# instance-based-loc/instance-based-loc

Hardware: AMD Instinct MI355X
Metric: query-frames localized/sec (embed+match+register) (higher is better)
Workload: dtype f16 (ViT MFMA operands, f32 accumulate) / f32+f64 (match, registration); 1 GPU; T: dinov2_vitb14 crops 224^2 (Q=7), 10000-instance memory (E=4), FPFH+RANSAC+coloured ICP on 5000-pt clouds, whole-memory evaluate; synthetic objects of extent U[0.15, 0.6] m on a 2.50 m grid (SURVEY 8d's U[0.2, 1.5] m re-scoped: its 5 000 points are too sparse to survive the radius-outlier removal); memory_instances=10000, points_per_object=5000, resident_feature_bytes_per_point=264, parallelism=frames-dp1+memory-replicated

## Files before the change

instance-based-loc_amd/csrc/reg_api.hip:

```cpp
#pragma clang fp contract(off)
#include <hip/hip_runtime.h>

#include <hipcub/hipcub.hpp>

#include <cctype>
#include <climits>
#include <cmath>
#include <cstdlib>
#include <cstring>
#include <string>
#include <vector>

#include "ibloc.h"
#include "reg_common.h"

#ifndef KNN_CELLS_NORMAL
#define KNN_CELLS_NORMAL 3.0
#endif
#ifndef KNN_CELLS_FEATURE
#define KNN_CELLS_FEATURE 5.0
#endif

#ifndef KNN_TILE_NORMAL
#define KNN_TILE_NORMAL 4
// ... 36 lines not shown
    bool auto0 = false;
};
static const DiagSwitch DIAG_SWITCHES[] = {
    {"knn_safety", nullptr},
    {"knn_rho", &RegDiag::knn_rho, 1, 4},
    {"knn_noguess", &RegDiag::knn_noguess},
    {"knn_debug", &RegDiag::knn_debug},
    {"feat_unfused", &RegDiag::feat_unfused},
    {"feat_valu", &RegDiag::feat_valu},
    {"feat_cand_cap", &RegDiag::feat_cand_cap, 1, INT_MAX, true},
    {"feat_p1_stride", &RegDiag::feat_p1_stride, 1},
    {"spfh_f64", &RegDiag::spfh_f64},
    {"spfh_qcap", &RegDiag::spfh_qcap, 1, INT_MAX, true},
    {"spfh_stats", &RegDiag::spfh_stats},
    {"eval_fullscan", &RegDiag::eval_fullscan},
    {"timing", &RegDiag::timing},
};

static const DiagSwitch* find_diag(const char* name) {
    for (const DiagSwitch& d : DIAG_SWITCHES)
        if (name && strcmp(name, d.name) == 0) return &d;
    return nullptr;
}

extern "C" int ibl_reg_ctx_set_diag(ibl_reg_ctx* ctx, const char* name, double value) {
    const DiagSwitch* d = find_diag(name);
    if (!ctx || !d || !std::isfinite(value)) return ibl_set_error(IBL_ERR_ARG, "ibl_reg_ctx_set_diag: null context, unknown switch or non-finite value");
    if (!d->field) ctx->diag.knn_safety = value;
    else if (d->auto0 && value == 0) ctx->diag.*d->field = 0;
    else ctx->diag.*d->field = (int)std::min(std::max(value, (double)d->lo), (double)d->hi);
// ... 381 lines not shown
```

instance-based-loc_amd/csrc/reg_common.h:

```cpp
#pragma once
#include <hip/hip_runtime.h>

#include <cstdint>

#include "ibl_common.h"

struct SegGrid {
    float minx, miny, minz, inv;
    int nx, ny, nz;
    int cell_base;
};

struct BatchGrid {
    const SegGrid* seg;
    const int* cell_start;
    const float4* sorted_pts;
    const int* order;
    int n_seg;
    const int* tile_base;
    const int* tile_seg;
    int n_tiles;
    int ts;
};

#define FM_P1_STRIDE 2

struct RegDiag {
    double knn_safety = 1.1;
    int knn_rho = 3;
    int knn_noguess = 0, knn_debug = 0;
    int feat_unfused = 0, feat_valu = 0, feat_cand_cap = 0;
    int feat_p1_stride = FM_P1_STRIDE;
    int spfh_f64 = 0, spfh_qcap = 0, spfh_stats = 0;
    int eval_fullscan = 0;
    int timing = 0;
};

struct ibl_reg_ctx {
    RegDiag diag;
    unsigned char* base = nullptr;
    int64_t size = 0;
    int64_t used = 0;
    int64_t high_water = 0;
    int device = 0;
    int* d_status = nullptr;
    unsigned char* pin = nullptr;
    int64_t pin_size = 0;
    int64_t pin_used = 0;
};
// ... 33 lines not shown
    } while (0)

#define IBL_ERR_ARENA (-5)
#define IBL_ERR_OVERFLOW (-6)

#define IBL_ST_GRID_OVERFLOW 1
#define IBL_ST_KNN_SLOWPATH 2
#define IBL_ST_FEAT_OVERFLOW 4
#define IBL_ST_RANSAC_OVERFLOW 8
#define IBL_ST_FEAT_REDONE 16
#define IBL_ST_RANSAC_REDONE 32

int ibl_build_batch_grid(ibl_reg_ctx* ctx, const float4* pts, const int* seg_off_dev, const int* seg_off_host, int n_seg,
                         float cell, int64_t max_cells, BatchGrid* out, hipStream_t s);
int ibl_build_batch_grid_bounded(ibl_reg_ctx* ctx, const float4* pts, const int* seg_off_dev, const int* seg_off_host, int n_seg,
                                 float cell, int64_t cells_bound, BatchGrid* out, hipStream_t s);
int ibl_build_tile_grid(ibl_reg_ctx* ctx, const float4* pts, const int* seg_off_dev, const int* seg_off_host, int n_seg,
                        const float* bbox_host, double radius, int max_nn, int ts, int64_t max_cells, BatchGrid* out, hipStream_t s);

int ibl_launch_bbox(const float4* pts, const int* seg_off_dev, int n_seg, float* bbox_dev, hipStream_t s);

struct FeatSources { const float4* normals[3]; const float* fpfh[3]; const float4* grad[3]; const unsigned short* split[3]; const float* norm[3]; };
struct FeatPair { int qkind, qsrc, qcnt, dkind, dsrc, dcnt, out, pad; };

int ibl_feat_search_mfma(ibl_reg_ctx* ctx, const FeatPair* d_pairs, int n_pairs, int max_q, const FeatSources& src, int* pair_idx,
                         float* pair_d2, const int* need_pos, const int* need_list, int out0, int64_t out_count, bool* overflow,
                         hipStream_t s);

int ibl_features_on_batch(ibl_reg_ctx* ctx, const float4* P, const int* seg_off_dev, const int* seg_off_host, int n_seg, const float* bbox_host, double voxel_size,
                          double grad_radius, int gq0, int gq1, float4* normals, float* fpfh, unsigned short* fpfh_split, float* fpfh_norm,
                          float4* grad, hipStream_t s);
// ... 173 lines not shown
```

instance-based-loc_amd/csrc/reg_grid.hip:

```cpp
#include <hip/hip_runtime.h>
#include <hipcub/hipcub.hpp>

#include <cstdlib>
#include <cstring>
#include <vector>

#include "reg_common.h"

__global__ __launch_bounds__(256) void ibl_bbox_kernel(const float4* __restrict__ pts, const int* __restrict__ seg_off,
                                                       float* __restrict__ bbox ) {
    const int s = blockIdx.x;
    const int b = seg_off[s], e = seg_off[s + 1];
    float mn[3] = {INFINITY, INFINITY, INFINITY}, mx[3] = {-INFINITY, -INFINITY, -INFINITY};
    for (int i = b + threadIdx.x; i < e; i += 256) {
        const float4 p = pts[i];
        mn[0] = fminf(mn[0], p.x); mn[1] = fminf(mn[1], p.y); mn[2] = fminf(mn[2], p.z);
        mx[0] = fmaxf(mx[0], p.x); mx[1] = fmaxf(mx[1], p.y); mx[2] = fmaxf(mx[2], p.z);
    }
    __shared__ float smn[3][256], smx[3][256];
    for (int a = 0; a < 3; ++a) { smn[a][threadIdx.x] = mn[a]; smx[a][threadIdx.x] = mx[a]; }
    __syncthreads();
    for (int st = 128; st >= 1; st >>= 1) {
        if (threadIdx.x < st)
            for (int a = 0; a < 3; ++a) {
// ... 21 lines not shown
    const float ex = b[3] - b[0], ey = b[4] - b[1], ez = b[5] - b[2];
    float c = cell;
    const float emax = fmaxf(ex, fmaxf(ey, ez));
    if (emax / 128.0f > c) c = emax / 128.0f;
    SegGrid g;
    g.minx = b[0]; g.miny = b[1]; g.minz = b[2];
    g.inv = 1.0f / c;
    g.nx = (int)floorf(ex * g.inv) + 1;
    g.ny = (int)floorf(ey * g.inv) + 1;
    g.nz = (int)floorf(ez * g.inv) + 1;
    g.cell_base = 0;
    return g;
}

__global__ __launch_bounds__(256) void ibl_grid_dims_kernel(const float* __restrict__ bbox, int n_seg, float cell, long long max_cells,
                                                            SegGrid* __restrict__ seg, int* __restrict__ total_cells, int* __restrict__ status) {
    __shared__ long long wave_sum[4];
    __shared__ long long carry;
    __shared__ int overflow_at;
    const int tid = threadIdx.x, lane = tid & 63, wave = tid >> 6;
    if (tid == 0) { carry = 0; overflow_at = -1; }
    __syncthreads();
    for (int base = 0; base < n_seg; base += 256) {
        const int s = base + tid;
        SegGrid g;
        long long cells = 0;
        if (s < n_seg) {
            g = seg_dims(bbox + s * 6, cell);
            cells = (long long)g.nx * g.ny * g.nz;
        }
        long long incl = cells;
#pragma unroll
        for (int off = 1; off < 64; off <<= 1) {
            const long long o = __shfl_up(incl, off, 64);
            if (lane >= off) incl += o;
        }
        if (lane == 63) wave_sum[wave] = incl;
        __syncthreads();
        long long before = carry;
        for (int w = 0; w < wave; ++w) before += wave_sum[w];
        const long long excl = before + incl - cells;
        if (s < n_seg) {
            if (excl + cells > max_cells) atomicMin(&overflow_at, s);
            g.cell_base = (int)excl;
            seg[s] = g;
        }
        __syncthreads();
        if (tid == 0) carry += wave_sum[0] + wave_sum[1] + wave_sum[2] + wave_sum[3];
        __syncthreads();
        if (overflow_at >= 0) break;
    }
    if (overflow_at >= 0) {
        if (tid == 0) {
            long long base = seg[overflow_at].cell_base;
            for (int s = overflow_at; s < n_seg; ++s) {
                SegGrid g = seg_dims(bbox + s * 6, cell);
                g.cell_base = (int)base;
                base += (long long)g.nx * g.ny * g.nz;
                if (base > max_cells) {
                    atomicOr(status, IBL_ST_GRID_OVERFLOW);
                    g.nx = g.ny = g.nz = 1;
                    base = g.cell_base + 1;
                }
                seg[s] = g;
            }
            *total_cells = (int)base;
        }
        return;
    }
    if (tid == 0) *total_cells = (int)carry;
}

__global__ __launch_bounds__(256) void ibl_cell_id_kernel(const float4* __restrict__ pts, const int* __restrict__ seg_off, int n_seg,
                                                          const SegGrid* __restrict__ seg, unsigned* __restrict__ keys,
                                                          int* __restrict__ vals, int* __restrict__ cell_count) {
    const int n = seg_off[n_seg];
    const int i = blockIdx.x * 256 + threadIdx.x;
    if (i >= n) return;
    const int s = seg_of(seg_off, n_seg, i);
    const SegGrid g = seg[s];
    const float4 p = pts[i];
    const int cx = cell_clamp(p.x, g.minx, g.inv, g.nx), cy = cell_clamp(p.y, g.miny, g.inv, g.ny),
              cz = cell_clamp(p.z, g.minz, g.inv, g.nz);
    const int c = g.cell_base + (cz * g.ny + cy) * g.nx + cx;
    keys[i] = (unsigned)c;
    vals[i] = i;
    atomicAdd(&cell_count[c], 1);
}

__global__ __launch_bounds__(256) void ibl_gather_sorted_kernel(const float4* __restrict__ pts, const int* __restrict__ order, int n,
                                                                float4* __restrict__ sorted) {
    const int i = blockIdx.x * 256 + threadIdx.x;
    if (i < n) sorted[i] = pts[order[i]];
}

static int grid_fill(ibl_reg_ctx* ctx, const float4* pts, const int* seg_off_dev, int n_seg, int n, const SegGrid* seg, int h_total,
                     BatchGrid* out, hipStream_t s) {
    int* cell_count; int* cell_start; unsigned *keys, *keys_out; int *vals, *order;
    float4* sorted;
    IBL_ARENA(cell_start, int, (int64_t)h_total + 2);
    IBL_ARENA(order, int, n + 1);
    IBL_ARENA(sorted, float4, n + 1);
    out->cell_start = cell_start; out->sorted_pts = sorted; out->order = order;
    ArenaMark scratch(ctx);
    IBL_ARENA(cell_count, int, (int64_t)h_total + 2);
    IBL_HIP_CHECK(hipMemsetAsync(cell_count, 0, sizeof(int) * (size_t)(h_total + 1), s));
    if (n == 0) {
        IBL_HIP_CHECK(hipMemsetAsync(cell_start, 0, sizeof(int) * (size_t)(h_total + 1), s));
        return IBL_OK;
    }
    IBL_ARENA(keys, unsigned, n);
    IBL_ARENA(keys_out, unsigned, n);
    IBL_ARENA(vals, int, n);
    hipLaunchKernelGGL(ibl_cell_id_kernel, dim3((n + 255) / 256), dim3(256), 0, s, pts, seg_off_dev, n_seg, seg, keys, vals,
                       cell_count);
    IBL_LAUNCH_CHECK();
    size_t tmp_scan = 0, tmp_sort = 0;
    IBL_HIP_CHECK(hipcub::DeviceScan::ExclusiveSum(nullptr, tmp_scan, cell_count, cell_start, h_total + 1, s));
// ... 12 lines not shown
int ibl_build_batch_grid(ibl_reg_ctx* ctx, const float4* pts, const int* seg_off_dev, const int* seg_off_host, int n_seg,
                         float cell, int64_t max_cells, BatchGrid* out, hipStream_t s) {
    const int n = seg_off_host[n_seg];
    float* bbox; SegGrid* seg; int* total;
    IBL_ARENA(bbox, float, (int64_t)n_seg * 6 + 6);
    IBL_ARENA(seg, SegGrid, n_seg + 1);
    IBL_ARENA(total, int, 4);
    out->seg = seg; out->cell_start = nullptr; out->sorted_pts = nullptr; out->order = nullptr; out->n_seg = n_seg;
    out->tile_base = nullptr; out->tile_seg = nullptr; out->n_tiles = 0; out->ts = 0;
    if (n_seg == 0) return IBL_OK;
    hipLaunchKernelGGL(ibl_bbox_kernel, dim3(n_seg), dim3(256), 0, s, pts, seg_off_dev, bbox);
    IBL_LAUNCH_CHECK();
    hipLaunchKernelGGL(ibl_grid_dims_kernel, dim3(1), dim3(256), 0, s, bbox, n_seg, cell, (long long)max_cells, seg, total,
                       ctx->d_status);
    IBL_LAUNCH_CHECK();
    int h_total = 0;
    IBL_HIP_CHECK(hipMemcpyAsync(&h_total, total, sizeof(int), hipMemcpyDeviceToHost, s));
    IBL_HIP_CHECK(hipStreamSynchronize(s));
    if (h_total <= 0 || h_total > max_cells) return ibl_set_error(IBL_ERR_OVERFLOW, "grid: %d cells exceed the budget %lld", h_total, (long long)max_cells);
    return grid_fill(ctx, pts, seg_off_dev, n_seg, n, seg, h_total, out, s);
}

int ibl_build_batch_grid_bounded(ibl_reg_ctx* ctx, const float4* pts, const int* seg_off_dev, const int* seg_off_host, int n_seg,
                                 float cell, int64_t cells_bound, BatchGrid* out, hipStream_t s) {
    const int n = seg_off_host[n_seg];
    float* bbox; SegGrid* seg; int* total;
    IBL_ARENA(bbox, float, (int64_t)n_seg * 6 + 6);
    IBL_ARENA(seg, SegGrid, n_seg + 1);
    IBL_ARENA(total, int, 4);
    out->seg = seg; out->cell_start = nullptr; out->sorted_pts = nullptr; out->order = nullptr; out->n_seg = n_seg;
    out->tile_base = nullptr; out->tile_seg = nullptr; out->n_tiles = 0; out->ts = 0;
    if (n_seg == 0) return IBL_OK;
    if (cells_bound <= 0 || cells_bound > 0x7fff0000ll) return ibl_set_error(IBL_ERR_OVERFLOW, "grid: cell bound %lld out of range", (long long)cells_bound);
    hipLaunchKernelGGL(ibl_bbox_kernel, dim3(n_seg), dim3(256), 0, s, pts, seg_off_dev, bbox);
    IBL_LAUNCH_CHECK();
    hipLaunchKernelGGL(ibl_grid_dims_kernel, dim3(1), dim3(256), 0, s, bbox, n_seg, cell, (long long)cells_bound, seg, total, ctx->d_status);
    IBL_LAUNCH_CHECK();
    return grid_fill(ctx, pts, seg_off_dev, n_seg, n, seg, (int)cells_bound, out, s);
}

int ibl_stage_upload(ibl_reg_ctx* ctx, void* dst_dev, const void* src_host, int64_t bytes, hipStream_t s) {
    if (bytes <= 0) return IBL_OK;
    const int64_t need = ibl_align_up(bytes, 64);
    if (ctx->pin && ctx->pin_used + need <= ctx->pin_size) {
        unsigned char* p = ctx->pin + ctx->pin_used;
        ctx->pin_used += need;
        memcpy(p, src_host, (size_t)bytes);
        IBL_HIP_CHECK(hipMemcpyAsync(dst_dev, p, (size_t)bytes, hipMemcpyHostToDevice, s));
        return IBL_OK;
    }
    IBL_HIP_CHECK(hipMemcpyAsync(dst_dev, src_host, (size_t)bytes, hipMemcpyHostToDevice, s));
    IBL_HIP_CHECK(hipStreamSynchronize(s));
    return IBL_OK;
// ... 4 lines not shown
    for (int t = tile_base[sgi] + threadIdx.x; t < tile_base[sgi + 1]; t += 256) tile_seg[t] = sgi;
}

int ibl_build_tile_grid(ibl_reg_ctx* ctx, const float4* pts, const int* seg_off_dev, const int* seg_off_host, int n_seg,
                        const float* bbox_host, double radius, int max_nn, int ts, int64_t max_cells, BatchGrid* out, hipStream_t s) {
    const int n = seg_off_host[n_seg];
    SegGrid* seg; int* tile_base;
    IBL_ARENA(seg, SegGrid, n_seg + 1);
    IBL_ARENA(tile_base, int, n_seg + 2);
    out->seg = seg; out->cell_start = nullptr; out->sorted_pts = nullptr; out->order = nullptr; out->n_seg = n_seg;
    out->tile_base = tile_base; out->tile_seg = nullptr; out->n_tiles = 0; out->ts = ts;
    if (n_seg == 0) return IBL_OK;
    std::vector<SegGrid> h(n_seg);
    std::vector<int> tb(n_seg + 1, 0);
    const double safety = ctx->diag.knn_safety, rho_t = (double)ctx->diag.knn_rho;
    long long cells = 0, tiles = 0;
    for (int sgi = 0; sgi < n_seg; ++sgi) {
        const float* b = bbox_host + 6 * (size_t)sgi;
        const float ex = b[3] - b[0], ey = b[4] - b[1], ez = b[5] - b[2];
        const int cnt = seg_off_host[sgi + 1] - seg_off_host[sgi];
        const double area = 2.0 * ((double)ex * ey + (double)ey * ez + (double)ez * ex);
        double c = radius;
        if (cnt > 0 && area > 0) {
            const double dens = (double)cnt / area;
            c = sqrt(safety * (double)max_nn / (3.141592653589793 * rho_t * rho_t * dens));
        }
        if (c > radius) c = radius;
        if (c < radius / 12.0) c = radius / 12.0;
        float cf = (float)c;
        const float emax = fmaxf(ex, fmaxf(ey, ez));
        if (emax / 128.0f > cf) cf = emax / 128.0f;
        SegGrid g;
        g.minx = b[0]; g.miny = b[1]; g.minz = b[2];
        g.inv = 1.0f / cf;
        g.nx = (int)floorf(ex * g.inv) + 1;
        g.ny = (int)floorf(ey * g.inv) + 1;
        g.nz = (int)floorf(ez * g.inv) + 1;
        if (cells + (long long)g.nx * g.ny * g.nz > max_cells) { g.nx = g.ny = g.nz = 1; }
        g.cell_base = (int)cells;
        cells += (long long)g.nx * g.ny * g.nz;
        h[sgi] = g;
        tb[sgi] = (int)tiles;
        tiles += (long long)((g.nx + ts - 1) / ts) * ((g.ny + ts - 1) / ts) * ((g.nz + ts - 1) / ts);
        if (tiles > 0x7fff0000ll) return ibl_set_error(IBL_ERR_OVERFLOW, "tile grid: too many tiles");
    }
    tb[n_seg] = (int)tiles;
    out->n_tiles = (int)tiles;
    int st = ibl_stage_upload(ctx, seg, h.data(), sizeof(SegGrid) * (int64_t)n_seg, s);
    if (st) return st;
    st = ibl_stage_upload(ctx, tile_base, tb.data(), sizeof(int) * (int64_t)(n_seg + 1), s);
    if (st) return st;
    if (tiles > 0) {
        int* tile_seg;
        IBL_ARENA(tile_seg, int, tiles + 1);
        hipLaunchKernelGGL(ibl_tile_seg_kernel, dim3(n_seg), dim3(256), 0, s, tile_base, tile_seg);
        IBL_LAUNCH_CHECK();
        out->tile_seg = tile_seg;
    }
    return grid_fill(ctx, pts, seg_off_dev, n_seg, n, seg, (int)cells, out, s);
}
```

instance-based-loc_amd/csrc/reg_icp.hip:

```cpp
#pragma clang fp contract(off)
#include <hip/hip_runtime.h>

#include <algorithm>
#include <cmath>

#include "ibloc.h"
#include "reg_common.h"
#include "reg_stages.h"

#ifndef ICP_GROUP_FROM
#define ICP_GROUP_FROM 8
#endif
#ifndef ICP_LPQ
#define ICP_LPQ 8
#endif
#define ICP_ACT_Y 32
static_assert(ICP_GROUP_FROM >= 1, "the first active-job list is written by the update of iteration ICP_GROUP_FROM - 1");
#define ICP_NACC 29

__global__ void ibl_icp_init_kernel(IcpState* __restrict__ st, int J, const RansacState* __restrict__ rs, int from_identity) {
    const int j = blockIdx.x * blockDim.x + threadIdx.x;
    if (j >= J) return;
    IcpState s;
    for (int i = 0; i < 16; ++i) s.T[i] = (from_identity || !rs) ? ((i % 5) == 0 ? 1.0 : 0.0) : rs[j].best_T[i];
// ... 176 lines not shown
    const float4 s4 = pts[i];
    double T[12], vs[3];
    for (int t = 0; t < 12; ++t) T[t] = S.T[t];
    xform_d(T, s4.x, s4.y, s4.z, vs);
    float d2 = r2;
    int pos = -1;
#pragma unroll 1
    for (int t = 0; t < 3; ++t) {
        const int k = J + 3 * j + t;
        if (piece_off[k + 1] > piece_off[k]) pos = nn_within(g, g.seg[k], (float)vs[0], (float)vs[1], (float)vs[2], radius, pos, &d2);
    }
    nn_idx[i] = pos >= 0 ? g.order[pos] : -1;
    nn_d2[i] = d2;
}

__global__ __launch_bounds__(256) void ibl_icp_step_kernel(const float4* __restrict__ pts, const float4* __restrict__ normals,
                                                           const float4* __restrict__ grad, const int* __restrict__ job_off, int J,
                                                           const IcpState* __restrict__ st, const int* __restrict__ nn_idx,
                                                           const float* __restrict__ nn_d2, int colored,
                                                           double sl_g, double sl_p, double* __restrict__ partial ,
                                                           const int* __restrict__ act_list, const int* __restrict__ act_cnt) {
    const int n_act = act_list ? *act_cnt : J;
    for (int a = blockIdx.y; a < n_act; a += gridDim.y) {
    const int j = act_list ? act_list[a] : a;
    const IcpState& S = st[j];
    if (S.done) continue;
    const int sb = job_off[j], se = job_off[j + 1];
    double T[12];
    for (int t = 0; t < 12; ++t) T[t] = S.T[t];
    double acc[ICP_NACC];
    for (int t = 0; t < ICP_NACC; ++t) acc[t] = 0.0;
    for (int i = sb + blockIdx.x * 256 + threadIdx.x; i < se; i += ICP_BPJ * 256) {
        const int tj = nn_idx[i];
        if (tj < 0) continue;
        const float d2 = nn_d2[i];
        const float4 s4 = pts[i];
        double vs[3];
        xform_d(T, s4.x, s4.y, s4.z, vs);
        acc[27] += 1.0;
        acc[28] += (double)d2;
        const float4 t4 = pts[tj];
        const double vt[3] = {t4.x, t4.y, t4.z};
        if (colored) {
            const float4 n4 = normals[tj], g4 = grad[tj];
// ... 23 lines not shown
        } else {
            for (int a = 0; a < 3; ++a) { acc[a] += vs[a]; acc[3 + a] += vt[a]; }
            for (int rr = 0; rr < 3; ++rr) for (int cc = 0; cc < 3; ++cc) acc[6 + 3 * rr + cc] += vt[rr] * vs[cc];
        }
    }
    __shared__ double sh[4][ICP_NACC];
    const int lane = threadIdx.x & 63, wave = threadIdx.x >> 6;
    for (int t = 0; t < ICP_NACC; ++t) {
        const double v = wave_sum_d(acc[t]);
        if (lane == 0) sh[wave][t] = v;
    }
    __syncthreads();
    if (threadIdx.x < ICP_NACC)
        partial[((int64_t)j * ICP_BPJ + blockIdx.x) * ICP_NACC + threadIdx.x] =
            ((sh[0][threadIdx.x] + sh[1][threadIdx.x]) + sh[2][threadIdx.x]) + sh[3][threadIdx.x];
    __syncthreads();
    }
}

__device__ inline bool solve6_d(double A[6][6], double* b, double* x) {
    double M[6][7];
    for (int i = 0; i < 6; ++i) { for (int j = 0; j < 6; ++j) M[i][j] = A[i][j]; M[i][6] = b[i]; }
    for (int c = 0; c < 6; ++c) {
        int piv = c;
        double mx = fabs(M[c][c]);
        for (int r = c + 1; r < 6; ++r) if (fabs(M[r][c]) > mx) { mx = fabs(M[r][c]); piv = r; }
        if (mx == 0.0 || !isfinite(mx)) return false;
        if (piv != c) for (int jj = 0; jj <= 6; ++jj) { const double t = M[c][jj]; M[c][jj] = M[piv][jj]; M[piv][jj] = t; }
        for (int r = c + 1; r < 6; ++r) {
            const double f = M[r][c] / M[c][c];
            for (int jj = c; jj <= 6; ++jj) M[r][jj] -= f * M[c][jj];
        }
    }
    for (int i = 5; i >= 0; --i) {
        double s = M[i][6];
        for (int jj = i + 1; jj < 6; ++jj) s -= M[i][jj] * x[jj];
        x[i] = s / M[i][i];
    }
    return true;
}

__device__ __forceinline__ void icp_update_job(IcpState* __restrict__ st, int j, const int* __restrict__ job_off, const double* __restrict__ partial,
                                               int colored, int max_iter, double rel_fitness, double rel_rmse, int* __restrict__ next_list,
                                               int* __restrict__ next_cnt);
__global__ __launch_bounds__(64) void ibl_icp_update_kernel(IcpState* __restrict__ st, int J, const int* __restrict__ job_off, const double* __restrict__ partial,
                                      int colored, int max_iter, double rel_fitness, double rel_rmse, const int* __restrict__ act_list,
                                      const int* __restrict__ act_cnt, int* __restrict__ next_list, int* __restrict__ next_cnt) {
    const int n_act = act_list ? *act_cnt : J;
    for (int a = blockIdx.x; a < n_act; a += gridDim.x)
        icp_update_job(st, act_list ? act_list[a] : a, job_off, partial, colored, max_iter, rel_fitness, rel_rmse, next_list, next_cnt);
}
__device__ __forceinline__ void icp_update_job(IcpState* __restrict__ st, int j, const int* __restrict__ job_off, const double* __restrict__ partial,
                                               int colored, int max_iter, double rel_fitness, double rel_rmse, int* __restrict__ next_list,
                                               int* __restrict__ next_cnt) {
    if (st[j].done) return;
    double mine = 0.0;
    if (threadIdx.x < ICP_NACC)
        for (int b = 0; b < ICP_BPJ; ++b) mine += partial[((int64_t)j * ICP_BPJ + b) * ICP_NACC + threadIdx.x];
    double a[ICP_NACC];
    for (int t = 0; t < ICP_NACC; ++t) a[t] = __shfl(mine, t, 64);
    if (threadIdx.x != 0) return;
    IcpState S = st[j];
    const int ns = job_off[j + 1] - job_off[j];
    const double cnt = a[27], err2 = a[28];
    const double nf = ns > 0 ? cnt / (double)ns : 0.0, nr = cnt > 0 ? sqrt(err2 / cnt) : 0.0;
    if (S.started && fabs(S.fitness - nf) < rel_fitness && fabs(S.rmse - nr) < rel_rmse) {
        S.fitness = nf; S.rmse = nr; S.done = 1;
        st[j] = S;
        return;
    }
    S.fitness = nf; S.rmse = nr; S.started = 1;
    if (S.iter >= max_iter) { S.done = 1; st[j] = S; return; }
    double U[16];
    for (int i = 0; i < 16; ++i) U[i] = (i % 5) == 0 ? 1.0 : 0.0;
    if (cnt > 0) {
        if (colored) {
            double A[6][6], nb[6], x[6];
            int q = 0;
            for (int r = 0; r < 6; ++r) for (int c = r; c < 6; ++c) { A[r][c] = a[q]; A[c][r] = a[q]; ++q; }
            for (int r = 0; r < 6; ++r) nb[r] = -a[21 + r];
            if (solve6_d(A, nb, x)) {
                const double ca = cos(x[0]), sa = sin(x[0]), cb = cos(x[1]), sb = sin(x[1]), cg = cos(x[2]), sg = sin(x[2]);
                U[0] = cg * cb; U[1] = cg * sb * sa - sg * ca; U[2] = cg * sb * ca + sg * sa; U[3] = x[3];
                U[4] = sg * cb; U[5] = sg * sb * sa + cg * ca; U[6] = sg * sb * ca - cg * sa; U[7] = x[4];
                U[8] = -sb;     U[9] = cb * sa;                U[10] = cb * ca;               U[11] = x[5];
            }
        } else {
            double sm[3], dm[3], H[3][3];
            for (int t = 0; t < 3; ++t) { sm[t] = a[t] / cnt; dm[t] = a[3 + t] / cnt; }
            for (int r = 0; r < 3; ++r) for (int c = 0; c < 3; ++c) H[r][c] = a[6 + 3 * r + c] - cnt * dm[r] * sm[c];
            kabsch_from_moments(sm, dm, H, U);
        }
    }
    double R[16];
    for (int r = 0; r < 4; ++r) for (int c = 0; c < 4; ++c) {
        double s = 0;
        for (int k = 0; k < 4; ++k) s += U[4 * r + k] * S.T[4 * k + c];
        R[4 * r + c] = s;
    }
    for (int i = 0; i < 16; ++i) S.T[i] = R[i];
    S.iter++;
    st[j] = S;
    if (next_list) next_list[atomicAdd(next_cnt, 1)] = j;
}

int ibl_reg_icp_stage(ibl_reg_ctx* ctx, RegPass& ps) {
    const int J = ps.J, colored = ps.colored ? 1 : 0;
    hipStream_t s = ps.s;
    const float radius = (float)ps.max_dist_icp, r2 = (float)(ps.max_dist_icp * ps.max_dist_icp);
    double* partial; int* icp_nn; float* icp_d2;
    IBL_ARENA(partial, double, (int64_t)J * ICP_BPJ * ICP_NACC);
    IBL_ARENA(icp_nn, int, ps.Ns + 64);
    IBL_ARENA(icp_d2, float, ps.Ns + 64);
    hipLaunchKernelGGL(ibl_icp_init_kernel, dim3((J + 63) / 64), dim3(64), 0, s, ps.is, J, ps.rs, colored ? 0 : 1);
    IBL_LAUNCH_CHECK();
    const double lambda_geometric = 0.968;
    const int max_iter = 30;
    int max_side = 0;
    for (int j = 0; j < J; ++j) max_side = std::max(max_side, ps.job_off[j + 1] - ps.job_off[j]);
    const unsigned chunks = (unsigned)std::max(1, (max_side + 255) / 256);
    int *act_list, *act_cnt;
    IBL_ARENA(act_list, int, 2 * (int64_t)J + 64);
    IBL_ARENA(act_cnt, int, max_iter + 8);
    IBL_HIP_CHECK(hipMemsetAsync(act_cnt, 0, sizeof(int) * (max_iter + 8), s));
    const unsigned act_y = (unsigned)std::min(J, ICP_ACT_Y);
    for (int it = 0; it <= max_iter; ++it) {
        const bool listed = it >= ICP_GROUP_FROM;
        const int* cur_list = listed ? act_list + (size_t)(it & 1) * J : nullptr;
        const int* cur_cnt = listed ? act_cnt + it : nullptr;
        int* nxt_list = it + 1 >= ICP_GROUP_FROM ? act_list + (size_t)((it + 1) & 1) * J : nullptr;
        int* nxt_cnt = it + 1 >= ICP_GROUP_FROM ? act_cnt + it + 1 : nullptr;
        if (!listed)
            hipLaunchKernelGGL(ibl_icp_nn_kernel, dim3(chunks, J), dim3(256), 0, s, ps.gC, ps.P, ps.d_job_off, J, ps.d_piece_off, ps.is, radius,
                               r2, icp_nn, icp_d2);
        else
            hipLaunchKernelGGL(ibl_icp_nn_group_kernel<ICP_LPQ>, dim3(chunks * ICP_LPQ, act_y), dim3(256), 0, s, ps.gC, ps.P, ps.d_job_off, J,
                               ps.d_piece_off, ps.is, radius, r2, icp_nn, icp_d2, cur_list, cur_cnt);
        IBL_LAUNCH_CHECK();
        hipLaunchKernelGGL(ibl_icp_step_kernel, dim3(ICP_BPJ, listed ? act_y : (unsigned)J), dim3(256), 0, s, ps.P, ps.normals, ps.grad, ps.d_job_off, J,
                           ps.is, icp_nn, icp_d2, colored, sqrt(lambda_geometric), sqrt(1.0 - lambda_geometric), partial, cur_list, cur_cnt);
        IBL_LAUNCH_CHECK();
        hipLaunchKernelGGL(ibl_icp_update_kernel, dim3(listed ? act_y : (unsigned)J), dim3(64), 0, s, ps.is, J, ps.d_job_off, partial, colored, max_iter,
                           1e-6, 1e-6, cur_list, cur_cnt, nxt_list, nxt_cnt);
        IBL_LAUNCH_CHECK();
    }
    return IBL_OK;
}
```

instance-based-loc_amd/csrc/reg_register.hip:

```cpp
#pragma clang fp contract(off)
#include <hip/hip_runtime.h>

#include <algorithm>
#include <cmath>
#include <cstdlib>
#include <ctime>
#include <vector>

#include "ibloc.h"
#include "reg_common.h"
#include "reg_stages.h"

#ifndef ICP_CELL_DIV
#define ICP_CELL_DIV 2.0
#endif


__global__ __launch_bounds__(256) void ibl_job_mean_kernel(const JobDesc* __restrict__ jobs, const float4* __restrict__ det,
                                                           const int* __restrict__ det_off, const float4* __restrict__ mem,
                                                           const int* __restrict__ mem_off, int center, double* __restrict__ means ) {
    const int j = blockIdx.x, side = blockIdx.y;
    const float4* pool = side == 0 ? det : mem;
    const int* off = side == 0 ? det_off : mem_off;
    double sx = 0, sy = 0, sz = 0;
// ... 89 lines not shown
    int st = ibl_stage_upload(ctx, ps.d_jobs, ps.jobs.data(), sizeof(JobDesc) * (int64_t)J, s);
    if (st) return st;
    st = ibl_stage_upload(ctx, ps.d_job_off, ps.job_off.data(), sizeof(int) * (int64_t)(2 * J + 1), s);
    if (st) return st;
    hipLaunchKernelGGL(ibl_job_mean_kernel, dim3(J, 2), dim3(256), 0, s, ps.d_jobs, ps.det, c.det_off_dev, ps.mem, c.mem_off_dev,
                       (c.flags & IBL_REG_CENTER) ? 1 : 0, ps.d_means);
    IBL_LAUNCH_CHECK();
    if (N > 0) {
        hipLaunchKernelGGL(ibl_job_gather_kernel, dim3((N + 255) / 256), dim3(256), 0, s, ps.d_jobs, J, ps.det, c.det_off_dev, ps.mem, c.mem_off_dev,
                           ps.d_job_off, ps.d_means, ps.P);
        IBL_LAUNCH_CHECK();
    }
    return IBL_OK;
}

static int64_t grid_c_cell_bound(const RegPass& ps, float cell0) {
    const RegCall& c = *ps.call;
    const int J = ps.J;
    int64_t bound = 0;
    for (int sgi = 0; sgi < 4 * J; ++sgi) {
        const int pl = sgi >= J ? 1 : 0, j = pl ? (sgi - J) / 3 : sgi, only = pl ? (sgi - J) % 3 : -1;
        float lo[3], hi[3];
        union_of_boxes(pl ? ps.jobs[j].tgt_seg : ps.jobs[j].src_seg, only, pl ? c.mem_off_host : c.det_off_host,
                       pl ? c.mem_features->bbox : c.det_features->bbox, lo, hi);
        double cells = 1;
        float cell = cell0;
        const float emax = std::max(hi[0] - lo[0], std::max(hi[1] - lo[1], hi[2] - lo[2]));
        if (emax * 1.0001f / 128.0f > cell) cell = emax / 128.0f;
        for (int a = 0; a < 3; ++a) cells *= std::floor((double)(hi[a] - lo[a]) * 1.0001 / cell) + 2.0;
        bound += (int64_t)cells;
    }
    return bound;
}

static int build_grid_c(ibl_reg_ctx* ctx, RegPass& ps) {
    const RegCall& c = *ps.call;
    const int J = ps.J;
    hipStream_t s = ps.s;
    const bool have = c.det_features && c.mem_features && c.det_features->bbox && c.mem_features->bbox;
    const int64_t budget = (int64_t)128 << 20;
    float cellC = (float)(ps.max_dist_icp / ICP_CELL_DIV);
    std::vector<int> piece_off(4 * (size_t)J + 1, 0);
    for (int j = 0; j <= J; ++j) piece_off[j] = ps.job_off[j];
    for (int j = 0; j < J; ++j)
        for (int t = 0; t < 3; ++t) {
            const int b = ps.jobs[j].tgt_seg[t];
            piece_off[J + 3 * j + t + 1] = piece_off[J + 3 * j + t] + (b >= 0 ? c.mem_off_host[b + 1] - c.mem_off_host[b] : 0);
        }
    IBL_ARENA(ps.d_piece_off, int, 4 * (int64_t)J + 1);
    int st = ibl_stage_upload(ctx, ps.d_piece_off, piece_off.data(), sizeof(int) * (4 * (int64_t)J + 1), s);
    if (st) return st;
    int64_t bound = have ? grid_c_cell_bound(ps, cellC) : 0;
    for (int tries = 0; have && bound >= budget && tries < 12; ++tries) { cellC *= 1.5f; bound = grid_c_cell_bound(ps, cellC); }
    if (have && bound < budget) return ibl_build_batch_grid_bounded(ctx, ps.P, ps.d_piece_off, piece_off.data(), 4 * J, cellC, bound, &ps.gC, s);
    for (int tries = 0; tries < 8; ++tries) {
        st = ibl_build_batch_grid(ctx, ps.P, ps.d_piece_off, piece_off.data(), 4 * J, cellC, budget, &ps.gC, s);
        if (st != IBL_ERR_OVERFLOW) break;
        cellC *= 2.0f;
    }
    return st;
}

enum { REDO_RANSAC_FULL_LIST = 1, REDO_FEAT_VALU = 2 };

static int read_back(ibl_reg_ctx* ctx, RegPass& ps, int* redo) {
    const RegCall& c = *ps.call;
    const int J = ps.J;
    hipStream_t s = ps.s;
    const RansacState* rs = ps.rs;
// ... 143 lines not shown
```

Baseline: 825.5 query-frames/s.

## Build spatial grids with one-pass per-segment LDS sort and fuse ICP update into step

Replaces the library radix-sort grid fill with a single kernel that bitonic-sorts (cell,index) keys per segment in shared memory and writes cell_start, order and sorted points directly, with tail blocks filling empty cells. Grid dims now also report the largest per-segment cell count so the host can check that keys fit in 32 bits. The ICP per-job update is moved into the step kernel (via an arrival counter), removing one launch per iteration. The aim is fewer launches and less sort overhead, at the cost of falling back when segments exceed the LDS cap and more complex last-block synchronisation.

Result: no change. 819.9 query-frames/s (median of 2 runs) (-0.7%).

```diff
diff --git a/instance-based-loc_amd/csrc/reg_api.hip b/instance-based-loc_amd/csrc/reg_api.hip
--- a/instance-based-loc_amd/csrc/reg_api.hip
+++ b/instance-based-loc_amd/csrc/reg_api.hip
@@ -74,6 +74,7 @@
     {"spfh_qcap", &RegDiag::spfh_qcap, 1, INT_MAX, true},
     {"spfh_stats", &RegDiag::spfh_stats},
     {"eval_fullscan", &RegDiag::eval_fullscan},
+    {"grid_lib_sort", &RegDiag::grid_lib_sort},
     {"timing", &RegDiag::timing},
 };
 
diff --git a/instance-based-loc_amd/csrc/reg_common.h b/instance-based-loc_amd/csrc/reg_common.h
--- a/instance-based-loc_amd/csrc/reg_common.h
+++ b/instance-based-loc_amd/csrc/reg_common.h
@@ -33,6 +33,7 @@
     int feat_p1_stride = FM_P1_STRIDE;
     int spfh_f64 = 0, spfh_qcap = 0, spfh_stats = 0;
     int eval_fullscan = 0;
+    int grid_lib_sort = 0;
     int timing = 0;
 };
 
@@ -96,7 +97,7 @@
 int ibl_build_batch_grid(ibl_reg_ctx* ctx, const float4* pts, const int* seg_off_dev, const int* seg_off_host, int n_seg,
                          float cell, int64_t max_cells, BatchGrid* out, hipStream_t s);
 int ibl_build_batch_grid_bounded(ibl_reg_ctx* ctx, const float4* pts, const int* seg_off_dev, const int* seg_off_host, int n_seg,
-                                 float cell, int64_t cells_bound, BatchGrid* out, hipStream_t s);
+                                 float cell, int64_t cells_bound, int64_t seg_cells_bound, BatchGrid* out, hipStream_t s);
 int ibl_build_tile_grid(ibl_reg_ctx* ctx, const float4* pts, const int* seg_off_dev, const int* seg_off_host, int n_seg,
                         const float* bbox_host, double radius, int max_nn, int ts, int64_t max_cells, BatchGrid* out, hipStream_t s);
 
diff --git a/instance-based-loc_amd/csrc/reg_grid.hip b/instance-based-loc_amd/csrc/reg_grid.hip
--- a/instance-based-loc_amd/csrc/reg_grid.hip
+++ b/instance-based-loc_amd/csrc/reg_grid.hip
@@ -1,6 +1,7 @@
 #include <hip/hip_runtime.h>
 #include <hipcub/hipcub.hpp>
 
+#include <algorithm>
 #include <cstdlib>
 #include <cstring>
 #include <vector>
@@ -59,12 +60,14 @@
 }
 
 __global__ __launch_bounds__(256) void ibl_grid_dims_kernel(const float* __restrict__ bbox, int n_seg, float cell, long long max_cells,
-                                                            SegGrid* __restrict__ seg, int* __restrict__ total_cells, int* __restrict__ status) {
+                                                            SegGrid* __restrict__ seg, int* __restrict__ total_cells ,
+                                                            int* __restrict__ status) {
     __shared__ long long wave_sum[4];
     __shared__ long long carry;
     __shared__ int overflow_at;
+    __shared__ int seg_max;
     const int tid = threadIdx.x, lane = tid & 63, wave = tid >> 6;
-    if (tid == 0) { carry = 0; overflow_at = -1; }
+    if (tid == 0) { carry = 0; overflow_at = -1; seg_max = 1; }
     __syncthreads();
     for (int base = 0; base < n_seg; base += 256) {
         const int s = base + tid;
@@ -73,6 +76,7 @@
         if (s < n_seg) {
             g = seg_dims(bbox + s * 6, cell);
             cells = (long long)g.nx * g.ny * g.nz;
+            atomicMax(&seg_max, (int)cells);
         }
         long long incl = cells;
 #pragma unroll
@@ -98,9 +102,11 @@
     if (overflow_at >= 0) {
         if (tid == 0) {
             long long base = seg[overflow_at].cell_base;
+            int mx = seg_max;
             for (int s = overflow_at; s < n_seg; ++s) {
                 SegGrid g = seg_dims(bbox + s * 6, cell);
                 g.cell_base = (int)base;
+                mx = max(mx, g.nx * g.ny * g.nz);
                 base += (long long)g.nx * g.ny * g.nz;
                 if (base > max_cells) {
                     atomicOr(status, IBL_ST_GRID_OVERFLOW);
@@ -109,11 +115,12 @@
                 }
                 seg[s] = g;
             }
-            *total_cells = (int)base;
+            total_cells[0] = (int)base;
+            total_cells[1] = mx;
         }
         return;
     }
-    if (tid == 0) *total_cells = (int)carry;
+    if (tid == 0) { total_cells[0] = (int)carry; total_cells[1] = seg_max; }
 }
 
 __global__ __launch_bounds__(256) void ibl_cell_id_kernel(const float4* __restrict__ pts, const int* __restrict__ seg_off, int n_seg,
@@ -139,14 +146,116 @@
     if (i < n) sorted[i] = pts[order[i]];
 }
 
-static int grid_fill(ibl_reg_ctx* ctx, const float4* pts, const int* seg_off_dev, int n_seg, int n, const SegGrid* seg, int h_total,
-                     BatchGrid* out, hipStream_t s) {
+#define GRID_LDS_CAP 16384
+#define GRID_TAIL_CHUNK 16384
+#define GRID_PAD_KEY 0xFFFFFFFFu
+
+__host__ __device__ static inline int grid_bits_for(unsigned count) {
+    int b = 0;
+    while (b < 32 && (1ull << b) < (unsigned long long)count) ++b;
+    return b;
+}
+
+__global__ __launch_bounds__(256) void ibl_grid_onepass_kernel(const float4* __restrict__ pts, const int* __restrict__ seg_off, int n_seg,
+                                                               const SegGrid* __restrict__ seg, int h_total, int lds_keys,
+                                                               int* __restrict__ cell_start, int* __restrict__ order,
+                                                               float4* __restrict__ sorted, int* __restrict__ status) {
+    extern __shared__ unsigned gkeys[];
+    const int tid = threadIdx.x, lane = tid & 63;
+    if ((int)blockIdx.x >= n_seg) {
+        const SegGrid gl = seg[n_seg - 1];
+        const long long first = (long long)gl.cell_base + (long long)gl.nx * gl.ny * gl.nz;
+        const long long c0 = (long long)(blockIdx.x - n_seg) * GRID_TAIL_CHUNK;
+        const long long lo = c0 > first ? c0 : first, hi = c0 + GRID_TAIL_CHUNK < (long long)h_total + 1 ? c0 + GRID_TAIL_CHUNK : (long long)h_total + 1;
+        const int n = seg_off[n_seg];
+        for (long long c = lo + tid; c < hi; c += 256) cell_start[c] = n;
+        return;
+    }
+    const int s = blockIdx.x;
+    const int b = seg_off[s], e = seg_off[s + 1], cnt = e - b;
+    const SegGrid g = seg[s];
+    const int ncell = g.nx * g.ny * g.nz;
+    const int ib = grid_bits_for((unsigned)cnt);
+    int n2 = 1;
+    while (n2 < cnt) n2 <<= 1;
+    if (n2 > lds_keys || ib + grid_bits_for((unsigned)ncell) > 32 || (long long)g.cell_base + ncell > (long long)h_total + 1) {
+        if (tid == 0) atomicOr(status, IBL_ST_GRID_OVERFLOW);
+        return;
+    }
+    for (int i = tid; i < n2; i += 256) {
+        unsigned key = GRID_PAD_KEY;
+        if (i < cnt) {
+            const float4 p = pts[b + i];
+            const int cx = cell_clamp(p.x, g.minx, g.inv, g.nx), cy = cell_clamp(p.y, g.miny, g.inv, g.ny),
+                      cz = cell_clamp(p.z, g.minz, g.inv, g.nz);
+            key = ((unsigned)((cz * g.ny + cy) * g.nx + cx) << ib) | (unsigned)i;
+        }
+        gkeys[i] = key;
+    }
+    __syncthreads();
+    for (int k = 2; k <= n2; k <<= 1)
+        for (int j = k >> 1; j > 0; j >>= 1) {
+            for (int t = tid; t < (n2 >> 1); t += 256) {
+                const int i = ((t & ~(j - 1)) << 1) | (t & (j - 1)), l = i | j;
+                const unsigned a = gkeys[i], c = gkeys[l];
+                if ((a > c) == ((i & k) == 0)) { gkeys[i] = c; gkeys[l] = a; }
+            }
+            __syncthreads();
+        }
+    const unsigned mask = (1u << ib) - 1u;
+    int* cs = cell_start + g.cell_base;
+    for (int p0 = tid - lane; p0 < cnt; p0 += 256) {
+        const int p = p0 + lane;
+        int c_first = 0, run = 0;
+        if (p < cnt) {
+            const unsigned key = gkeys[p];
+            const int i = b + (int)(key & mask), c = (int)(key >> ib), c_prev = p > 0 ? (int)(gkeys[p - 1] >> ib) : -1;
+            order[b + p] = i;
+            sorted[b + p] = pts[i];
+            c_first = c_prev + 1;
+            run = c - c_prev;
+            if (run <= 2) {
+                for (int q = 0; q < run; ++q) cs[c_first + q] = b + p;
+                run = 0;
+            }
+        }
+        for (unsigned long long m = __ballot(run > 0); m != 0ull; m &= m - 1ull) {
+            const int src = __ffsll((long long)m) - 1;
+            const int cf = __shfl(c_first, src, 64), rn = __shfl(run, src, 64);
+            for (int q = lane; q < rn; q += 64) cs[cf + q] = b + p0 + src;
+        }
+    }
+    const int c_last = cnt > 0 ? (int)(gkeys[cnt - 1] >> ib) : -1;
+    for (int c = c_last + 1 + tid; c < ncell; c += 256) cs[c] = e;
+}
+
+static bool grid_onepass_fits(const int* seg_off_host, int n_seg, int64_t seg_cells_bound, int* lds_keys) {
+    int max_cnt = 0;
+    for (int s = 0; s < n_seg; ++s) max_cnt = std::max(max_cnt, seg_off_host[s + 1] - seg_off_host[s]);
+    if (max_cnt > GRID_LDS_CAP || seg_cells_bound < 1 || seg_cells_bound > 0x7fffffffll) return false;
+    if (grid_bits_for((unsigned)max_cnt) + grid_bits_for((unsigned)seg_cells_bound) > 32) return false;
+    int n2 = 1;
+    while (n2 < max_cnt) n2 <<= 1;
+    *lds_keys = n2;
+    return true;
+}
+
+static int grid_fill(ibl_reg_ctx* ctx, const float4* pts, const int* seg_off_dev, const int* seg_off_host, int n_seg, int n,
+                     const SegGrid* seg, int h_total, int64_t seg_cells_bound, BatchGrid* out, hipStream_t s) {
     int* cell_count; int* cell_start; unsigned *keys, *keys_out; int *vals, *order;
     float4* sorted;
     IBL_ARENA(cell_start, int, (int64_t)h_total + 2);
     IBL_ARENA(order, int, n + 1);
     IBL_ARENA(sorted, float4, n + 1);
     out->cell_start = cell_start; out->sorted_pts = sorted; out->order = order;
+    int lds_keys = 0;
+    if (!ctx->diag.grid_lib_sort && grid_onepass_fits(seg_off_host, n_seg, seg_cells_bound, &lds_keys)) {
+        const unsigned tail = (unsigned)(((int64_t)h_total + 1 + GRID_TAIL_CHUNK - 1) / GRID_TAIL_CHUNK);
+        hipLaunchKernelGGL(ibl_grid_onepass_kernel, dim3((unsigned)n_seg + tail), dim3(256), sizeof(unsigned) * (size_t)lds_keys, s, pts,
+                           seg_off_dev, n_seg, seg, h_total, lds_keys, cell_start, order, sorted, ctx->d_status);
+        IBL_LAUNCH_CHECK();
+        return IBL_OK;
+    }
     ArenaMark scratch(ctx);
     IBL_ARENA(cell_count, int, (int64_t)h_total + 2);
     IBL_HIP_CHECK(hipMemsetAsync(cell_count, 0, sizeof(int) * (size_t)(h_total + 1), s));
@@ -189,15 +298,16 @@
     hipLaunchKernelGGL(ibl_grid_dims_kernel, dim3(1), dim3(256), 0, s, bbox, n_seg, cell, (long long)max_cells, seg, total,
                        ctx->d_status);
     IBL_LAUNCH_CHECK();
-    int h_total = 0;
-    IBL_HIP_CHECK(hipMemcpyAsync(&h_total, total, sizeof(int), hipMemcpyDeviceToHost, s));
+    int h_tot[2] = {0, 0};
+    IBL_HIP_CHECK(hipMemcpyAsync(h_tot, total, sizeof(h_tot), hipMemcpyDeviceToHost, s));
     IBL_HIP_CHECK(hipStreamSynchronize(s));
+    const int h_total = h_tot[0];
     if (h_total <= 0 || h_total > max_cells) return ibl_set_error(IBL_ERR_OVERFLOW, "grid: %d cells exceed the budget %lld", h_total, (long long)max_cells);
-    return grid_fill(ctx, pts, seg_off_dev, n_seg, n, seg, h_total, out, s);
+    return grid_fill(ctx, pts, seg_off_dev, seg_off_host, n_seg, n, seg, h_total, h_tot[1], out, s);
 }
 
 int ibl_build_batch_grid_bounded(ibl_reg_ctx* ctx, const float4* pts, const int* seg_off_dev, const int* seg_off_host, int n_seg,
-                                 float cell, int64_t cells_bound, BatchGrid* out, hipStream_t s) {
+                                 float cell, int64_t cells_bound, int64_t seg_cells_bound, BatchGrid* out, hipStream_t s) {
     const int n = seg_off_host[n_seg];
     float* bbox; SegGrid* seg; int* total;
     IBL_ARENA(bbox, float, (int64_t)n_seg * 6 + 6);
@@ -211,7 +321,7 @@
     IBL_LAUNCH_CHECK();
     hipLaunchKernelGGL(ibl_grid_dims_kernel, dim3(1), dim3(256), 0, s, bbox, n_seg, cell, (long long)cells_bound, seg, total, ctx->d_status);
     IBL_LAUNCH_CHECK();
-    return grid_fill(ctx, pts, seg_off_dev, n_seg, n, seg, (int)cells_bound, out, s);
+    return grid_fill(ctx, pts, seg_off_dev, seg_off_host, n_seg, n, seg, (int)cells_bound, seg_cells_bound, out, s);
 }
 
 int ibl_stage_upload(ibl_reg_ctx* ctx, void* dst_dev, const void* src_host, int64_t bytes, hipStream_t s) {
@@ -246,7 +356,7 @@
     std::vector<SegGrid> h(n_seg);
     std::vector<int> tb(n_seg + 1, 0);
     const double safety = ctx->diag.knn_safety, rho_t = (double)ctx->diag.knn_rho;
-    long long cells = 0, tiles = 0;
+    long long cells = 0, tiles = 0, seg_cells = 1;
     for (int sgi = 0; sgi < n_seg; ++sgi) {
         const float* b = bbox_host + 6 * (size_t)sgi;
         const float ex = b[3] - b[0], ey = b[4] - b[1], ez = b[5] - b[2];
@@ -271,6 +381,7 @@
         if (cells + (long long)g.nx * g.ny * g.nz > max_cells) { g.nx = g.ny = g.nz = 1; }
         g.cell_base = (int)cells;
         cells += (long long)g.nx * g.ny * g.nz;
+        seg_cells = std::max(seg_cells, (long long)g.nx * g.ny * g.nz);
         h[sgi] = g;
         tb[sgi] = (int)tiles;
         tiles += (long long)((g.nx + ts - 1) / ts) * ((g.ny + ts - 1) / ts) * ((g.nz + ts - 1) / ts);
@@ -289,5 +400,5 @@
         IBL_LAUNCH_CHECK();
         out->tile_seg = tile_seg;
     }
-    return grid_fill(ctx, pts, seg_off_dev, n_seg, n, seg, (int)cells, out, s);
-}
+    return grid_fill(ctx, pts, seg_off_dev, seg_off_host, n_seg, n, seg, (int)cells, seg_cells, out, s);
+}
diff --git a/instance-based-loc_amd/csrc/reg_icp.hip b/instance-based-loc_amd/csrc/reg_icp.hip
--- a/instance-based-loc_amd/csrc/reg_icp.hip
+++ b/instance-based-loc_amd/csrc/reg_icp.hip
@@ -214,20 +214,98 @@
     nn_d2[i] = d2;
 }
 
-__global__ __launch_bounds__(256) void ibl_icp_step_kernel(const float4* __restrict__ pts, const float4* __restrict__ normals,
+__device__ inline bool solve6_d(double A[6][6], double* b, double* x) {
+    double M[6][7];
+    for (int i = 0; i < 6; ++i) { for (int j = 0; j < 6; ++j) M[i][j] = A[i][j]; M[i][6] = b[i]; }
+    for (int c = 0; c < 6; ++c) {
+        int piv = c;
+        double mx = fabs(M[c][c]);
+        for (int r = c + 1; r < 6; ++r) if (fabs(M[r][c]) > mx) { mx = fabs(M[r][c]); piv = r; }
+        if (mx == 0.0 || !isfinite(mx)) return false;
+        if (piv != c) for (int jj = 0; jj <= 6; ++jj) { const double t = M[c][jj]; M[c][jj] = M[piv][jj]; M[piv][jj] = t; }
+        for (int r = c + 1; r < 6; ++r) {
+            const double f = M[r][c] / M[c][c];
+            for (int jj = c; jj <= 6; ++jj) M[r][jj] -= f * M[c][jj];
+        }
+    }
+    for (int i = 5; i >= 0; --i) {
+        double s = M[i][6];
+        for (int jj = i + 1; jj < 6; ++jj) s -= M[i][jj] * x[jj];
+        x[i] = s / M[i][i];
+    }
+    return true;
+}
+
+__device__ __attribute__((noinline)) void icp_update_job(IcpState* st, int j, const int* __restrict__ job_off, const double* partial, int colored,
+                                               int max_iter, double rel_fitness, double rel_rmse, int* __restrict__ next_list,
+                                               int* __restrict__ next_cnt) {
+    const int lane = threadIdx.x;
+    double mine = 0.0;
+    if (lane < ICP_NACC)
+        for (int b = 0; b < ICP_BPJ; ++b) mine += partial[((int64_t)j * ICP_BPJ + b) * ICP_NACC + lane];
+    double a[ICP_NACC];
+    for (int t = 0; t < ICP_NACC; ++t) a[t] = __shfl(mine, t, 64);
+    if (lane != 0) return;
+    IcpState S = st[j];
+    const int ns = job_off[j + 1] - job_off[j];
+    const double cnt = a[27], err2 = a[28];
+    const double nf = ns > 0 ? cnt / (double)ns : 0.0, nr = cnt > 0 ? sqrt(err2 / cnt) : 0.0;
+    if (S.started && fabs(S.fitness - nf) < rel_fitness && fabs(S.rmse - nr) < rel_rmse) {
+        S.fitness = nf; S.rmse = nr; S.done = 1;
+        st[j] = S;
+        return;
+    }
+    S.fitness = nf; S.rmse = nr; S.started = 1;
+    if (S.iter >= max_iter) { S.done = 1; st[j] = S; return; }
+    double U[16];
+    for (int i = 0; i < 16; ++i) U[i] = (i % 5) == 0 ? 1.0 : 0.0;
+    if (cnt > 0) {
+        if (colored) {
+            double A[6][6], nb[6], x[6];
+            int q = 0;
+            for (int r = 0; r < 6; ++r) for (int c = r; c < 6; ++c) { A[r][c] = a[q]; A[c][r] = a[q]; ++q; }
+            for (int r = 0; r < 6; ++r) nb[r] = -a[21 + r];
+            if (solve6_d(A, nb, x)) {
+                const double ca = cos(x[0]), sa = sin(x[0]), cb = cos(x[1]), sb = sin(x[1]), cg = cos(x[2]), sg = sin(x[2]);
+                U[0] = cg * cb; U[1] = cg * sb * sa - sg * ca; U[2] = cg * sb * ca + sg * sa; U[3] = x[3];
+                U[4] = sg * cb; U[5] = sg * sb * sa + cg * ca; U[6] = sg * sb * ca - cg * sa; U[7] = x[4];
+                U[8] = -sb;     U[9] = cb * sa;                U[10] = cb * ca;               U[11] = x[5];
+            }
+        } else {
+            double sm[3], dm[3], H[3][3];
+            for (int t = 0; t < 3; ++t) { sm[t] = a[t] / cnt; dm[t] = a[3 + t] / cnt; }
+            for (int r = 0; r < 3; ++r) for (int c = 0; c < 3; ++c) H[r][c] = a[6 + 3 * r + c] - cnt * dm[r] * sm[c];
+            kabsch_from_moments(sm, dm, H, U);
+        }
+    }
+    double R[16];
+    for (int r = 0; r < 4; ++r) for (int c = 0; c < 4; ++c) {
+        double s = 0;
+        for (int k = 0; k < 4; ++k) s += U[4 * r + k] * S.T[4 * k + c];
+        R[4 * r + c] = s;
+    }
+    for (int i = 0; i < 16; ++i) S.T[i] = R[i];
+    S.iter++;
+    st[j] = S;
+    if (next_list) next_list[atomicAdd(next_cnt, 1)] = j;
+}
+
+__global__ __launch_bounds__(256, 2) void ibl_icp_step_kernel(const float4* __restrict__ pts, const float4* __restrict__ normals,
                                                            const float4* __restrict__ grad, const int* __restrict__ job_off, int J,
-                                                           const IcpState* __restrict__ st, const int* __restrict__ nn_idx,
+                                                           IcpState* st, const int* __restrict__ nn_idx,
                                                            const float* __restrict__ nn_d2, int colored,
-                                                           double sl_g, double sl_p, double* __restrict__ partial ,
-                                                           const int* __restrict__ act_list, const int* __restrict__ act_cnt) {
+                                                           double sl_g, double sl_p, double* partial ,
+                                                           const int* __restrict__ act_list, const int* __restrict__ act_cnt,
+                                                           int* __restrict__ arrived , int max_iter,
+                                                           double rel_fitness, double rel_rmse, int* __restrict__ next_list,
+                                                           int* __restrict__ next_cnt) {
     const int n_act = act_list ? *act_cnt : J;
     for (int a = blockIdx.y; a < n_act; a += gridDim.y) {
     const int j = act_list ? act_list[a] : a;
-    const IcpState& S = st[j];
-    if (S.done) continue;
+    if (st[j].done) continue;
     const int sb = job_off[j], se = job_off[j + 1];
     double T[12];
-    for (int t = 0; t < 12; ++t) T[t] = S.T[t];
+    for (int t = 0; t < 12; ++t) T[t] = st[j].T[t];
     double acc[ICP_NACC];
     for (int t = 0; t < ICP_NACC; ++t) acc[t] = 0.0;
     for (int i = sb + blockIdx.x * 256 + threadIdx.x; i < se; i += ICP_BPJ * 256) {
@@ -281,94 +359,18 @@
     if (threadIdx.x < ICP_NACC)
         partial[((int64_t)j * ICP_BPJ + blockIdx.x) * ICP_NACC + threadIdx.x] =
             ((sh[0][threadIdx.x] + sh[1][threadIdx.x]) + sh[2][threadIdx.x]) + sh[3][threadIdx.x];
+    if (threadIdx.x < 64) {
+        __threadfence();
+        int last = 0;
+        if (threadIdx.x == 0) last = atomicAdd(&arrived[j], 1) == ICP_BPJ - 1;
+        if (__shfl(last, 0, 64)) {
+            __threadfence();
+            if (threadIdx.x == 0) arrived[j] = 0;
+            icp_update_job(st, j, job_off, partial, colored, max_iter, rel_fitness, rel_rmse, next_list, next_cnt);
+        }
+    }
     __syncthreads();
     }
-}
-
-__device__ inline bool solve6_d(double A[6][6], double* b, double* x) {
-    double M[6][7];
-    for (int i = 0; i < 6; ++i) { for (int j = 0; j < 6; ++j) M[i][j] = A[i][j]; M[i][6] = b[i]; }
-    for (int c = 0; c < 6; ++c) {
-        int piv = c;
-        double mx = fabs(M[c][c]);
-        for (int r = c + 1; r < 6; ++r) if (fabs(M[r][c]) > mx) { mx = fabs(M[r][c]); piv = r; }
-        if (mx == 0.0 || !isfinite(mx)) return false;
-        if (piv != c) for (int jj = 0; jj <= 6; ++jj) { const double t = M[c][jj]; M[c][jj] = M[piv][jj]; M[piv][jj] = t; }
-        for (int r = c + 1; r < 6; ++r) {
-            const double f = M[r][c] / M[c][c];
-            for (int jj = c; jj <= 6; ++jj) M[r][jj] -= f * M[c][jj];
-        }
-    }
-    for (int i = 5; i >= 0; --i) {
-        double s = M[i][6];
-        for (int jj = i + 1; jj < 6; ++jj) s -= M[i][jj] * x[jj];
-        x[i] = s / M[i][i];
-    }
-    return true;
-}
-
-__device__ __forceinline__ void icp_update_job(IcpState* __restrict__ st, int j, const int* __restrict__ job_off, const double* __restrict__ partial,
-                                               int colored, int max_iter, double rel_fitness, double rel_rmse, int* __restrict__ next_list,
-                                               int* __restrict__ next_cnt);
-__global__ __launch_bounds__(64) void ibl_icp_update_kernel(IcpState* __restrict__ st, int J, const int* __restrict__ job_off, const double* __restrict__ partial,
-                                      int colored, int max_iter, double rel_fitness, double rel_rmse, const int* __restrict__ act_list,
-                                      const int* __restrict__ act_cnt, int* __restrict__ next_list, int* __restrict__ next_cnt) {
-    const int n_act = act_list ? *act_cnt : J;
-    for (int a = blockIdx.x; a < n_act; a += gridDim.x)
-        icp_update_job(st, act_list ? act_list[a] : a, job_off, partial, colored, max_iter, rel_fitness, rel_rmse, next_list, next_cnt);
-}
-__device__ __forceinline__ void icp_update_job(IcpState* __restrict__ st, int j, const int* __restrict__ job_off, const double* __restrict__ partial,
-                                               int colored, int max_iter, double rel_fitness, double rel_rmse, int* __restrict__ next_list,
-                                               int* __restrict__ next_cnt) {
-    if (st[j].done) return;
-    double mine = 0.0;
-    if (threadIdx.x < ICP_NACC)
-        for (int b = 0; b < ICP_BPJ; ++b) mine += partial[((int64_t)j * ICP_BPJ + b) * ICP_NACC + threadIdx.x];
-    double a[ICP_NACC];
-    for (int t = 0; t < ICP_NACC; ++t) a[t] = __shfl(mine, t, 64);
-    if (threadIdx.x != 0) return;
-    IcpState S = st[j];
-    const int ns = job_off[j + 1] - job_off[j];
-    const double cnt = a[27], err2 = a[28];
-    const double nf = ns > 0 ? cnt / (double)ns : 0.0, nr = cnt > 0 ? sqrt(err2 / cnt) : 0.0;
-    if (S.started && fabs(S.fitness - nf) < rel_fitness && fabs(S.rmse - nr) < rel_rmse) {
-        S.fitness = nf; S.rmse = nr; S.done = 1;
-        st[j] = S;
-        return;
-    }
-    S.fitness = nf; S.rmse = nr; S.started = 1;
-    if (S.iter >= max_iter) { S.done = 1; st[j] = S; return; }
-    double U[16];
-    for (int i = 0; i < 16; ++i) U[i] = (i % 5) == 0 ? 1.0 : 0.0;
-    if (cnt > 0) {
-        if (colored) {
-            double A[6][6], nb[6], x[6];
-            int q = 0;
-            for (int r = 0; r < 6; ++r) for (int c = r; c < 6; ++c) { A[r][c] = a[q]; A[c][r] = a[q]; ++q; }
-            for (int r = 0; r < 6; ++r) nb[r] = -a[21 + r];
-            if (solve6_d(A, nb, x)) {
-                const double ca = cos(x[0]), sa = sin(x[0]), cb = cos(x[1]), sb = sin(x[1]), cg = cos(x[2]), sg = sin(x[2]);
-                U[0] = cg * cb; U[1] = cg * sb * sa - sg * ca; U[2] = cg * sb * ca + sg * sa; U[3] = x[3];
-                U[4] = sg * cb; U[5] = sg * sb * sa + cg * ca; U[6] = sg * sb * ca - cg * sa; U[7] = x[4];
-                U[8] = -sb;     U[9] = cb * sa;                U[10] = cb * ca;               U[11] = x[5];
-            }
-        } else {
-            double sm[3], dm[3], H[3][3];
-            for (int t = 0; t < 3; ++t) { sm[t] = a[t] / cnt; dm[t] = a[3 + t] / cnt; }
-            for (int r = 0; r < 3; ++r) for (int c = 0; c < 3; ++c) H[r][c] = a[6 + 3 * r + c] - cnt * dm[r] * sm[c];
-            kabsch_from_moments(sm, dm, H, U);
-        }
-    }
-    double R[16];
-    for (int r = 0; r < 4; ++r) for (int c = 0; c < 4; ++c) {
-        double s = 0;
-        for (int k = 0; k < 4; ++k) s += U[4 * r + k] * S.T[4 * k + c];
-        R[4 * r + c] = s;
-    }
-    for (int i = 0; i < 16; ++i) S.T[i] = R[i];
-    S.iter++;
-    st[j] = S;
-    if (next_list) next_list[atomicAdd(next_cnt, 1)] = j;
 }
 
 int ibl_reg_icp_stage(ibl_reg_ctx* ctx, RegPass& ps) {
@@ -387,9 +389,11 @@
     for (int j = 0; j < J; ++j) max_side = std::max(max_side, ps.job_off[j + 1] - ps.job_off[j]);
     const unsigned chunks = (unsigned)std::max(1, (max_side + 255) / 256);
     int *act_list, *act_cnt;
+    const int n_cnt = (max_iter + 8 + 3) & ~3;
     IBL_ARENA(act_list, int, 2 * (int64_t)J + 64);
-    IBL_ARENA(act_cnt, int, max_iter + 8);
-    IBL_HIP_CHECK(hipMemsetAsync(act_cnt, 0, sizeof(int) * (max_iter + 8), s));
+    IBL_ARENA(act_cnt, int, n_cnt + (int64_t)J + 4);
+    int* arrived = act_cnt + n_cnt;
+    IBL_HIP_CHECK(hipMemsetAsync(act_cnt, 0, sizeof(int) * (size_t)(n_cnt + ((J + 3) & ~3)), s));
     const unsigned act_y = (unsigned)std::min(J, ICP_ACT_Y);
     for (int it = 0; it <= max_iter; ++it) {
         const bool listed = it >= ICP_GROUP_FROM;
@@ -405,11 +409,9 @@
                                ps.d_piece_off, ps.is, radius, r2, icp_nn, icp_d2, cur_list, cur_cnt);
         IBL_LAUNCH_CHECK();
         hipLaunchKernelGGL(ibl_icp_step_kernel, dim3(ICP_BPJ, listed ? act_y : (unsigned)J), dim3(256), 0, s, ps.P, ps.normals, ps.grad, ps.d_job_off, J,
-                           ps.is, icp_nn, icp_d2, colored, sqrt(lambda_geometric), sqrt(1.0 - lambda_geometric), partial, cur_list, cur_cnt);
+                           ps.is, icp_nn, icp_d2, colored, sqrt(lambda_geometric), sqrt(1.0 - lambda_geometric), partial, cur_list, cur_cnt,
+                           arrived, max_iter, 1e-6, 1e-6, nxt_list, nxt_cnt);
         IBL_LAUNCH_CHECK();
-        hipLaunchKernelGGL(ibl_icp_update_kernel, dim3(listed ? act_y : (unsigned)J), dim3(64), 0, s, ps.is, J, ps.d_job_off, partial, colored, max_iter,
-                           1e-6, 1e-6, cur_list, cur_cnt, nxt_list, nxt_cnt);
-        IBL_LAUNCH_CHECK();
     }
     return IBL_OK;
 }
diff --git a/instance-based-loc_amd/csrc/reg_register.hip b/instance-based-loc_amd/csrc/reg_register.hip
--- a/instance-based-loc_amd/csrc/reg_register.hip
+++ b/instance-based-loc_amd/csrc/reg_register.hip
@@ -127,10 +127,11 @@
     return IBL_OK;
 }
 
-static int64_t grid_c_cell_bound(const RegPass& ps, float cell0) {
+static int64_t grid_c_cell_bound(const RegPass& ps, float cell0, int64_t* seg_bound) {
     const RegCall& c = *ps.call;
     const int J = ps.J;
     int64_t bound = 0;
+    *seg_bound = 1;
     for (int sgi = 0; sgi < 4 * J; ++sgi) {
         const int pl = sgi >= J ? 1 : 0, j = pl ? (sgi - J) / 3 : sgi, only = pl ? (sgi - J) % 3 : -1;
         float lo[3], hi[3];
@@ -142,6 +143,7 @@
         if (emax * 1.0001f / 128.0f > cell) cell = emax / 128.0f;
         for (int a = 0; a < 3; ++a) cells *= std::floor((double)(hi[a] - lo[a]) * 1.0001 / cell) + 2.0;
         bound += (int64_t)cells;
+        *seg_bound = std::max(*seg_bound, (int64_t)cells);
     }
     return bound;
 }
@@ -163,9 +165,11 @@
     IBL_ARENA(ps.d_piece_off, int, 4 * (int64_t)J + 1);
     int st = ibl_stage_upload(ctx, ps.d_piece_off, piece_off.data(), sizeof(int) * (4 * (int64_t)J + 1), s);
     if (st) return st;
-    int64_t bound = have ? grid_c_cell_bound(ps, cellC) : 0;
-    for (int tries = 0; have && bound >= budget && tries < 12; ++tries) { cellC *= 1.5f; bound = grid_c_cell_bound(ps, cellC); }
-    if (have && bound < budget) return ibl_build_batch_grid_bounded(ctx, ps.P, ps.d_piece_off, piece_off.data(), 4 * J, cellC, bound, &ps.gC, s);
+    int64_t seg_bound = 1;
+    int64_t bound = have ? grid_c_cell_bound(ps, cellC, &seg_bound) : 0;
+    for (int tries = 0; have && bound >= budget && tries < 12; ++tries) { cellC *= 1.5f; bound = grid_c_cell_bound(ps, cellC, &seg_bound); }
+    if (have && bound < budget)
+        return ibl_build_batch_grid_bounded(ctx, ps.P, ps.d_piece_off, piece_off.data(), 4 * J, cellC, bound, seg_bound, &ps.gC, s);
     for (int tries = 0; tries < 8; ++tries) {
         st = ibl_build_batch_grid(ctx, ps.P, ps.d_piece_off, piece_off.data(), 4 * J, cellC, budget, &ps.gC, s);
         if (st != IBL_ERR_OVERFLOW) break;
```
